# veronicaguerrini/BFQzip

Measured on AMD Instinct MI355X. Metric: Mbases/s end-to-end (eBWT+cluster+LF), reads and results resident in HBM, higher is better.
Workload: dtype u64

## Files before the change

### bfqzip_amd/_lib.py

```python
import ctypes as C
import os
import subprocess

_HERE = os.path.dirname(os.path.abspath(__file__))
LIB_PATH = os.path.join(_HERE, "libbfqhip.so")
_LIB = None

SYMBOLS = [
    "bfq_default_params", "bfq_create", "bfq_create_error", "bfq_destroy", "bfq_set_params",
    "bfq_last_error", "bfq_stream", "bfq_device_count", "bfq_pick_device", "bfq_device_lease", "bfq_device_release",
    "bfq_phase_enable", "bfq_phase", "bfq_phase_report", "bfq_output_prefault", "bfq_fastq_rows_estimate", "bfq_build_ebwt", "bfq_count_reads",
    "bfq_smooth_invert", "bfq_run_reads", "bfq_run_reads_device", "bfq_fetch_ebwt",
    "bfq_fastq_out_bound", "bfq_fastq_build_ebwt", "bfq_fastq_run", "bfq_fastq_run_streams",
    "bfq_smooth_invert_fastq", "bfq_fastq_run_job", "bfq_host_alloc", "bfq_host_free",
    "bfq_text_count_lines", "bfq_text_nth_newline", "bfq_file_put", "bfq_file_map", "bfq_file_unmap", "bfq_fastq_build_ebwt_fd", "bfq_smooth_invert_fastq_fd",
    "bfq_glob_begin", "bfq_glob_local_text", "bfq_glob_pile_counts", "bfq_glob_init_out", "bfq_glob_run_pile", "bfq_glob_finish",
    "bfq_synth_default", "bfq_synth_total", "bfq_synth_host", "bfq_synth_device", "bfq_synth_fastq",
    "bfq_posbin_geometry", "bfq_radix_geometry", "bfq_refine_form", "bfq_prof_enable", "bfq_prof_reset", "bfq_prof_count", "bfq_prof_get", "bfq_prof_trace_select", "bfq_prof_trace",
    "bfq_stream_bound", "bfq_stream_raw_len", "bfq_stream_compress", "bfq_stream_decompress",
    "bfq_stream_reserve", "bfq_stream_compress_device", "bfq_stream_ebwt_decode",
    "bfq_names_compress", "bfq_names_compress_device",
    "bfq_quals_compress", "bfq_quals_compress_device",
    "bfq_fastq_restore_bound", "bfq_fastq_restore", "bfq_fastq_restore_fd",
    "bfq_reorder_key", "bfq_fastq_reorder", "bfq_fastq_reorder_fd",
    "bfq_perm_bound", "bfq_perm_reads", "bfq_perm_encode", "bfq_perm_decode",
    "bfq_fastq_reorder_keep", "bfq_fastq_reorder_keep_fd", "bfq_fastq_unreorder", "bfq_fastq_unreorder_fd",
    "bfq_fastq_restore_ordered", "bfq_fastq_restore_ordered_fd",
    "bfq_fastq_restore_groups", "bfq_stream_members", "bfq_fastq_restore_grouped", "bfq_fastq_restore_grouped_fd",
    "bfq_fastq_compare", "bfq_fastq_compare_fd",
    "bfq_bgzf_probe", "bfq_bgzf_index", "bfq_bgzf_inflate", "bfq_bgzf_inflate_device", "bfq_bgzf_inflate_fd",
    "bfq_bgzf_deflate_bound", "bfq_bgzf_deflate_host", "bfq_bgzf_deflate", "bfq_bgzf_deflate_device", "bfq_bgzf_deflate_fd",
    "bfq_fastq_restore_bgzf_fd",
    "bfq_gzip_probe", "bfq_gzip_measure", "bfq_gzip_inflate", "bfq_gzip_inflate_device", "bfq_gzip_inflate_fd", "bfq_gzip_inflate_host",
    "bfq_gzip_host_error",
    "bfq_bam_default_opts", "bfq_bam_probe", "bfq_bam_measure", "bfq_bam_to_fastq", "bfq_bam_to_fastq_device", "bfq_bam_to_fastq_fd",
    "bfq_bam_to_fastq_host", "bfq_bam_host_error",
    "bfq_bam_patch_host", "bfq_bam_patch_device", "bfq_bam_patch", "bfq_bam_patch_fd",
    "bfq_ubam_default_opts", "bfq_fastq_to_bam_measure", "bfq_fastq_to_bam_host", "bfq_ubam_host_error", "bfq_fastq_to_bam_device", "bfq_fastq_to_bam",
    "bfq_fastq_to_bam_fd", "bfq_fastq_restore_bam_fd",
    "bfq_pairs_default_opts", "bfq_pairs_host_error",
    "bfq_fastq_deinterleave_measure", "bfq_fastq_deinterleave", "bfq_fastq_deinterleave_device", "bfq_fastq_deinterleave_fd", "bfq_fastq_deinterleave_host",
    "bfq_fastq_interleave_measure", "bfq_fastq_interleave", "bfq_fastq_interleave_device", "bfq_fastq_interleave_fd", "bfq_fastq_interleave_host",
    "bfq_repair_default_opts", "bfq_fastq_repair_measure", "bfq_fastq_repair", "bfq_fastq_repair_device", "bfq_fastq_repair_fd", "bfq_fastq_repair_host",
    "bfq_workspace_bytes", "bfq_workspace_read", "bfq_version",
]


class Params(C.Structure):
    _fields_ = [(k, C.c_int32) for k in ("K", "m", "v", "f", "t", "term", "M", "B", "ext", "piles", "ws_cap_mib")] + \
               [("reserved", C.c_int32 * 5)]

# ... 352 lines not shown
        L.bfq_fastq_to_bam_measure.argtypes = [vp, C.POINTER(vp), a3, puo, pu64, a3, pus]
        L.bfq_fastq_to_bam_host.argtypes = [C.POINTER(vp), a3, puo, vp, u64, pu64, pus]
        L.bfq_fastq_to_bam_device.argtypes = [vp, C.POINTER(vp), a3, puo, vp, u64, pu64, pus]
        L.bfq_fastq_to_bam.argtypes = [vp, C.POINTER(vp), a3, puo, vp, u64, pu64, pus]
        L.bfq_fastq_to_bam_fd.argtypes = [vp, i3, puo, C.c_int, pu64, pus]
        L.bfq_fastq_restore_bam_fd.argtypes = [vp, C.c_int, u64, C.c_int, u64, C.c_int, u64, C.c_int, u64, puo, C.c_int, pu64, pus]
        ppo, pps2 = C.POINTER(PairsOpts), C.POINTER(PairsStats)
        L.bfq_pairs_default_opts.restype = None
        L.bfq_pairs_default_opts.argtypes = [ppo]
        L.bfq_pairs_host_error.restype = C.c_char_p
        L.bfq_pairs_host_error.argtypes = []
        L.bfq_fastq_deinterleave_measure.argtypes = [vp, vp, u64, ppo, a3, a3, pps2]
        L.bfq_fastq_deinterleave.argtypes = [vp, vp, u64, ppo, C.POINTER(vp), a3, a3, a3, pps2]
        L.bfq_fastq_deinterleave_device.argtypes = [vp, vp, u64, ppo, C.POINTER(vp), a3, a3, a3, pps2]
        L.bfq_fastq_deinterleave_fd.argtypes = [vp, C.c_int, u64, ppo, i3, a3, a3, pps2]
        L.bfq_fastq_deinterleave_host.argtypes = [vp, u64, ppo, C.POINTER(vp), a3, a3, a3, pps2]
        L.bfq_fastq_interleave_measure.argtypes = [vp, C.POINTER(vp), a3, ppo, pu64, a3, pps2]
        L.bfq_fastq_interleave.argtypes = [vp, C.POINTER(vp), a3, ppo, vp, u64, pu64, pps2]
        L.bfq_fastq_interleave_device.argtypes = [vp, C.POINTER(vp), a3, ppo, vp, u64, pu64, pps2]
        L.bfq_fastq_interleave_fd.argtypes = [vp, i3, ppo, C.c_int, pu64, pps2]
        L.bfq_fastq_interleave_host.argtypes = [C.POINTER(vp), a3, ppo, vp, u64, pu64, pps2]
        pro, prs = C.POINTER(RepairOpts), C.POINTER(RepairStats)
        L.bfq_repair_default_opts.restype = None
        L.bfq_repair_default_opts.argtypes = [pro]
        L.bfq_fastq_repair_measure.argtypes = [vp, C.POINTER(vp), a3, pro, a3, a3, prs]
        L.bfq_fastq_repair.argtypes = [vp, C.POINTER(vp), a3, pro, C.POINTER(vp), a3, a3, a3, prs]
        L.bfq_fastq_repair_device.argtypes = [vp, C.POINTER(vp), a3, pro, C.POINTER(vp), a3, a3, a3, prs]
        L.bfq_fastq_repair_fd.argtypes = [vp, i3, pro, i3, a3, a3, prs]
        L.bfq_fastq_repair_host.argtypes = [C.POINTER(vp), a3, pro, C.POINTER(vp), a3, a3, a3, prs]
        L.bfq_fastq_restore_bgzf_fd.argtypes = [vp, C.c_int, u64, C.c_int, u64, C.c_int, u64, C.c_int, u64, C.c_int, C.c_int, pu64, pu64, pu64]
        L.bfq_posbin_geometry.argtypes = [u64, C.POINTER(u64), C.POINTER(C.c_int)]
        L.bfq_radix_geometry.argtypes = [u64, C.POINTER(u64), C.POINTER(u64)]
        L.bfq_refine_form.argtypes = [vp]
        L.bfq_prof_enable.argtypes = [vp, C.c_int]
        L.bfq_prof_reset.argtypes = [vp]
        L.bfq_prof_count.argtypes = [vp]
        L.bfq_prof_trace_select.argtypes = [vp, C.c_int]
        L.bfq_prof_trace.restype = C.c_int64
        L.bfq_prof_trace.argtypes = [vp, vp, u64]
        L.bfq_prof_get.argtypes = [vp, C.c_int, C.c_char_p, C.c_int, C.POINTER(C.c_double),
                                   C.POINTER(u64), C.POINTER(C.c_double)]
        _LIB = L
    return _LIB
```

### bfqzip_amd/api.py

```python
import ctypes as C
import numpy as np
from . import _lib


class BfqError(RuntimeError):
    def __init__(self, code, msg):
        super().__init__(f"libbfqhip error {code}: {msg}")
        self.code = code


def make_params(k=16, m=2, v=ord(">"), f=40, t=20, s=ord("#"), M=2, B=0, ext=0, piles=0, ws_cap_mib=0):
    p = _lib.Params()
    p.K, p.m, p.v, p.f, p.t, p.term, p.M, p.B, p.ext, p.piles, p.ws_cap_mib = k, m, v, f, t, s, M, B, ext, piles, ws_cap_mib
    return p


def _ptr(a):
    return C.c_void_p(a.ctypes.data) if a is not None else None


def _u8(text):
    if isinstance(text, np.ndarray):
        return text if (text.dtype == np.uint8 and text.flags.c_contiguous) else np.ascontiguousarray(text, np.uint8)
    return np.frombuffer(text, np.uint8)
# ... 1270 lines not shown

    @staticmethod
    def perm_encode(perm, mode=0, k=0, seed=0):
        return perm_encode(perm, mode=mode, k=k, seed=seed)

    @staticmethod
    def perm_decode(permz):
        return perm_decode(permz)

    def stream_compress_device(self, d_in, n, d_out, cap):
        ol = C.c_uint64(0)
        self._ck(self.L.bfq_stream_compress_device(self.h, d_in, n, d_out, cap, C.byref(ol)))
        return int(ol.value)

    def names_compress_device(self, d_in, n, d_out, cap, always=False):
        ol = C.c_uint64(0)
        self._ck(self.L.bfq_names_compress_device(self.h, d_in, n, 1 if always else 0, d_out, cap, C.byref(ol)))
        return int(ol.value)

    def quals_compress_device(self, d_in, n, d_out, cap, always=False, rung=None):
        ol = C.c_uint64(0)
        self._ck(self.L.bfq_quals_compress_device(self.h, d_in, n, self._quals_flags(always, rung), d_out, cap, C.byref(ol)))
        return int(ol.value)

    def stream_reserve(self, n):
        self._ck(self.L.bfq_stream_reserve(self.h, n))

    def stream_bound(self, n):
        return int(self.L.bfq_stream_bound(n))

    def refine_form(self):
        return int(self.L.bfq_refine_form(self.h))

    def prof_reset(self):
        self.L.bfq_prof_reset(self.h)

    def prof(self):
        out = {}
        name = C.create_string_buffer(64)
        for i in range(self.L.bfq_prof_count(self.h)):
            ms = C.c_double(); ln = C.c_uint64(); by = C.c_double()
            self.L.bfq_prof_get(self.h, i, name, 64, C.byref(ms), C.byref(ln), C.byref(by))
            if ln.value:
                out[name.value.decode()] = {"ms": ms.value, "launches": ln.value, "alg_bytes": by.value}
        return out

    def prof_trace_select(self, kernel):
        name = C.create_string_buffer(64)
        idx = -1
        for i in range(self.L.bfq_prof_count(self.h)):
            self.L.bfq_prof_get(self.h, i, name, 64, None, None, None)
            if kernel is not None and name.value.decode() == kernel:
                idx = i
        if kernel is not None and idx < 0:
            raise KeyError(kernel)
        self._ck(self.L.bfq_prof_trace_select(self.h, idx))

    def prof_trace(self):
        k = int(self.L.bfq_prof_trace(self.h, None, 0))
        out = np.empty(max(k, 0), np.float32)
        if k > 0:
            self.L.bfq_prof_trace(self.h, _ptr(out), k)
        return out

    def workspace_bytes(self):
        return int(self.L.bfq_workspace_bytes(self.h))
# ... 74 lines not shown
```

### bfqzip_amd/csrc/bfq_api.hip

```cpp
#include <math.h>
#include <time.h>
#include <stdlib.h>
#include <stdio.h>
#include <string.h>
#include <unistd.h>
#include <errno.h>
#include <algorithm>
#include <new>
#include "bfq_internal.h"
#include "bfq_synth.h"
#include "bfq_device.h"
#include "bfq_rank.h"
#include "bfq_posbin.h"

const char *const BFQ_KERNEL_NAMES[K_NUM] = {
    "k_text_from_reads", "k_pack3", "k_build_keys", "k_radix_hist", "k_scan", "k_radix_scatter", "k_huge_round",
    "k_cluster_big", "k_refine_chunk", "k_refine_big", "k_emit_bwt", "k_lf_count", "k_lf_build", "k_lcp_flags",
    "k_cluster", "k_invert_count", "k_invert", "k_synth", "k_fastq", "k_bfs", "k_codec", "misc",
    "k_restore_index", "k_fq_format_lines", "k_reorder_keys", "k_reorder_gather",
    "k_fq_format_ordered", "k_perm_pack", "k_perm_invert", "k_posbin_l1", "k_posbin_l2", "k_posbin_apply", "k_posbin_check",
    "k_cmp_check", "k_cmp_compare", "k_cmp_emit", "k_bgzf_inflate", "k_bgzf_deflate", "k_ubam_size", "k_ubam_write", "k_pairs_cmp", "k_pairs_move"};

static thread_local std::string g_createErr;

// ... 240 lines not shown
    if (!c) return;
    memset(c->profMs, 0, sizeof c->profMs); memset(c->profLaunches, 0, sizeof c->profLaunches);
    memset(c->profBytes, 0, sizeof c->profBytes);
    c->profTrace.clear();
}
extern "C" int bfq_prof_trace_select(bfq_ctx *c, int idx)
{
    if (!c || idx < -1 || idx >= K_NUM) return BFQ_E_ARG;
    c->profTraceId = idx; c->profTrace.clear();
    return BFQ_OK;
}
extern "C" int64_t bfq_prof_trace(bfq_ctx *c, float *ms, uint64_t cap)
{
    if (!c) return BFQ_E_ARG;
    const size_t k = std::min<size_t>(cap, c->profTrace.size());
    if (ms && k) memcpy(ms, c->profTrace.data(), k * sizeof(float));
    return (int64_t)c->profTrace.size();
}
extern "C" int bfq_prof_count(bfq_ctx *c) { (void)c; return K_NUM; }
extern "C" int bfq_posbin_geometry(uint64_t n_rows, uint64_t *window, int *bin_shift)
{
    const int s = bfq_posbin_shift(n_rows);
    if (window) *window = BFQ_PB_W;
    if (bin_shift) *bin_shift = s;
    return s >= 0 ? BFQ_OK : BFQ_E_ARG;
}
extern "C" int bfq_radix_geometry(uint64_t n_rows, uint64_t *tile_rows, uint64_t *block_rows)
{
    if (tile_rows) *tile_rows = BFQ_RS_TILE;
    if (block_rows) *block_rows = bfq_radix_block_elems(n_rows);
    return BFQ_OK;
}
extern "C" int bfq_refine_form(bfq_ctx *c) { return c ? (c->env.refinePipe ? 1 : 0) : BFQ_E_ARG; }
extern "C" int bfq_prof_get(bfq_ctx *c, int idx, char *name, int cap, double *ms, uint64_t *launches, double *bytes)
{
    if (!c || idx < 0 || idx >= K_NUM) return BFQ_E_ARG;
    if (name && cap > 0) { strncpy(name, BFQ_KERNEL_NAMES[idx], cap - 1); name[cap - 1] = 0; }
    if (ms) *ms = c->profMs[idx];
    if (launches) *launches = c->profLaunches[idx];
    if (bytes) *bytes = c->profBytes[idx];
    return BFQ_OK;
}

static void check_counters(bfq_ctx *c)
{
    const DevCounters &h = c->h_cnt;
    if (h.errSymbol) throw BfqError{BFQ_E_SYMBOL, "symbol outside {A,C,G,T,N,terminator}"};
    if (h.errTooLong) throw BfqError{BFQ_E_TOO_LONG, "read longer than BFQ_MAX_READ_LEN"};
    if (h.errInvert) throw BfqError{BFQ_E_NOT_EBWT, "LF walk did not close: not an eBWT of a read collection"};
    if (h.mismatch) throw BfqError{BFQ_E_NOT_EBWT, "eBWT is not in #_i<#_j<A<C<G<N<T suffix order"};
    if (h.errFreq3) throw BfqError{BFQ_E_FREQ3, "three frequent symbols in a cluster (bfq_int.cpp:505 assert); raise -f"};
}
static void finish_call(bfq_ctx *c, bfq_stats *st = nullptr)
{
    c->fetchCounters();
    c->profCollect();
    check_counters(c);
    if (!st) return;
    const u64 *s = c->h_cnt.stats;
    st->num_clust = s[0]; st->num_clust_discarded = s[1]; st->num_clust_amb_discarded = s[2];
    st->num_clust_mod = s[3]; st->num_clust_alleq = s[4]; st->bases_inside = s[5];
    st->qs_smoothed = s[6]; st->modified = s[7];
    st->n_rows = c->n; st->n_reads = c->N;
    st->n_segments = c->h_cnt.nSegs; st->n_big_segments = c->h_cnt.bigTotal + c->h_cnt.bigCount;
}

// ... 1258 lines not shown
```

### bfqzip_amd/csrc/bfq_host.cpp

```cpp
#include <errno.h>
#include <fcntl.h>
#include <stdio.h>
#include <stdlib.h>
#include <string.h>
#include <sched.h>
#include <sys/file.h>
#include <sys/mman.h>
#include <sys/stat.h>
#include <time.h>
#include <unistd.h>
#include <algorithm>
#include <atomic>
#include <condition_variable>
#include <mutex>
#include <string>
#include <thread>
#include <vector>
#include "bfq_internal_host.h"
#include "bfq_reorder.h"
#include "bfq_perm.h"
#include "bfq_bgzf.h"

static double now_s()
{
    struct timespec ts;
    clock_gettime(CLOCK_MONOTONIC, &ts);
    return ts.tv_sec + 1e-9 * ts.tv_nsec;
}

BfqEnv bfq_env_read()
{
    {
        BfqEnv e;
        auto geti = [](const char *k, int dflt) { const char *v = getenv(k); return (v && *v) ? atoi(v) : dflt; };
        auto getu = [](const char *k, unsigned long long dflt) {
            const char *v = getenv(k);
            if (!v || !*v) return dflt;
            char *end = nullptr;
            double x = strtod(v, &end);
            if (end && (*end == 'G' || *end == 'g')) x *= 1073741824.0;
            else if (end && (*end == 'M' || *end == 'm')) x *= 1048576.0;
            else if (end && (*end == 'K' || *end == 'k')) x *= 1024.0;
            return (unsigned long long)x;
        };
        e.trace = getenv("BFQ_TRACE") != nullptr;
        e.piles = getenv("BFQ_PILES") ? (atoi(getenv("BFQ_PILES")) == 2 ? 2 : atoi(getenv("BFQ_PILES")) ? 1 : -1) : 0;
        e.pilesSplit = getenv("BFQ_PILES_SPLIT") != nullptr;
        e.noOverlap = getenv("BFQ_NO_OVERLAP") != nullptr;
        e.noLengthGuess = getenv("BFQ_NO_LENGTH_GUESS") != nullptr;
        e.posMode = geti("BFQ_POSMODE", 0) != 0;
        e.posBins = geti("BFQ_POSBINS", 1) != 0;
        e.posBinWc = geti("BFQ_POSBIN_WC", 1) != 0;
        e.fuseKeys = geti("BFQ_FUSEKEYS", 1) != 0;
        e.refinePipe = geti("BFQ_REFINE_PIPE", 1) != 0;
        e.ioThreads = geti("BFQ_IO_THREADS", 0);
        e.prefaultThreads = geti("BFQ_PREFAULT_THREADS", -1);
        e.hugeCap = getu("BFQ_HUGE_CAP", 0);
        e.wsCap = getu("BFQ_WS_CAP", 0);
        e.device = getenv("BFQ_DEVICE") ? atoi(getenv("BFQ_DEVICE")) : -1;
        e.fakeDevices = geti("BFQ_FAKE_DEVICES", 0);
        e.lease = geti("BFQ_LEASE", 1) != 0;
        if (const char *d = getenv("BFQ_LEASE_DIR")) e.leaseDir = d;
        e.noOutmap = getenv("BFQ_NO_OUTMAP") != nullptr;
        e.compact = geti("BFQ_COMPACT", 0) != 0;
        if (const char *v = getenv("BFQ_POISON")) {
            char *end = nullptr;
            const long b = strtol(v, &end, 0);
            if (*v && end && !*end && b >= 0 && b <= 255) e.poison = (int)b;
        }
        e.prefaultPause = geti("BFQ_PREFAULT_PAUSE", 0) != 0;
        e.compactWin = getu("BFQ_COMPACT_WIN", 0);
        e.compactRing = getu("BFQ_COMPACT_RING", 0);
        e.bgzfBatch = getu("BFQ_BGZF_BATCH", 0);
        e.dnaStatic = geti("BFQ_DNA_STATIC", 0);
        e.dnacK = geti("BFQ_DNAC_K", 0); e.dnacH = geti("BFQ_DNAC_H", 0); e.dnacW = geti("BFQ_DNAC_W", 0); e.dnacSkip = geti("BFQ_DNAC_TSKIP", -1);
        return e;
    }
}
const BfqEnv &bfq_env()
{
    static const BfqEnv E = bfq_env_read();
    return E;
}

int bfq_cpu_budget()
{
    static const int budget = [] {
// ... 523 lines not shown
```

### bfqzip_amd/csrc/bfq_internal_host.h

```cpp
#pragma once
#include <stdint.h>
#include <sys/mman.h>
#include <atomic>
#include <new>
#include <string>
#include "../../include/bfqzip_hip.h"
#include "bfq_common.h"

struct BfqError {
    int code;
    std::string msg;
};

template <class F> static int host_guarded(std::string &err, F body)
{
    err.clear();
    try {
        body();
        return BFQ_OK;
    } catch (const BfqError &e) {
        err = e.msg;
        return e.code;
    } catch (const std::bad_alloc &) {
        err = "host out of memory";
        return BFQ_E_NOMEM;
    }
}
static inline void zero3(uint64_t *a) { if (a) a[0] = a[1] = a[2] = 0; }

struct MappedInput {
    void *p = MAP_FAILED; size_t n = 0;
    MappedInput() = default;
    MappedInput(const MappedInput &) = delete; MappedInput &operator=(const MappedInput &) = delete;
    bool open(int fd, size_t len) { n = len; p = len ? mmap(nullptr, len, PROT_READ, MAP_PRIVATE, fd, 0) : MAP_FAILED; return !len || p != MAP_FAILED; }
    const uint8_t *data() const { return p != MAP_FAILED ? (const uint8_t *)p : nullptr; }
    ~MappedInput() { if (p != MAP_FAILED) munmap(p, n); }
};

struct BfqEnv {
    bool trace = false;
    int piles = 0;
    bool pilesSplit = false;
    bool noOverlap = false;
    bool noLengthGuess = false;
    bool posMode = false;
    bool posBins = true;
    bool posBinWc = true;
    bool fuseKeys = true;
    bool refinePipe = true;
    int ioThreads = 0;
    int prefaultThreads = -1;
    unsigned long long hugeCap = 0;
    unsigned long long wsCap = 0;
    int device = -1;
    int fakeDevices = 0;
    bool lease = true;
    std::string leaseDir;
    bool compact = false;
    int dnaStatic = 0;
    int dnacK = 0, dnacH = 0, dnacW = 0, dnacSkip = -1;
    unsigned long long compactRing = 0;
    unsigned long long compactWin = 0;
    bool prefaultPause = false;
    unsigned long long bgzfBatch = 0;
    int poison = -1;
    bool noOutmap = false;
};
BfqEnv bfq_env_read();
const BfqEnv &bfq_env();
int bfq_cpu_budget();
extern std::atomic<bool> g_bfqHipStarted;
extern std::atomic<int> g_bfqUploadsRunning;

struct bfq_outmap;
bfq_outmap *bfq_outmap_open(int fd, uint64_t map_len, uint64_t prefault_len);
bfq_outmap *bfq_outmap_take(int fd, uint64_t min_len);
char *bfq_outmap_ptr(bfq_outmap *m);
uint64_t bfq_outmap_len(bfq_outmap *m);
void bfq_outmap_extend(bfq_outmap *m, uint64_t prefault_len);
bool bfq_outmap_close(bfq_outmap *m, uint64_t final_len);
bool bfq_outmap_ensure(bfq_outmap *m, uint64_t off, uint64_t len);
int bfq_outmap_fd(bfq_outmap *m);
// ... 9 lines not shown
```

### bfqzip_amd/csrc/k_cluster.hip

```cpp
#include <stdlib.h>
#include "bfq_internal.h"
#include "bfq_device.h"
#include "bfq_rank.h"
#include "bfq_rankblk.h"

__global__ __launch_bounds__(256) void k_lcp_flags(const u16 *__restrict__ lcp, u64 n, int K, u8 *__restrict__ in)
{
    const u64 ngroups = (n + 7) / 8;
    for (u64 g = (u64)blockIdx.x * blockDim.x + threadIdx.x; g < ngroups; g += (u64)gridDim.x * blockDim.x) {
        u64 r0 = g * 8;
        int l[10];
        if (r0 >= 1 && r0 + 9 <= n) {
            u64 a = *(const u64 *)(lcp + r0 - 1), b = *(const u64 *)(lcp + r0 + 3);
            u32 c = *(const u32 *)(lcp + r0 + 7);
#pragma unroll
            for (int k = 0; k < 4; k++) { l[k] = (int)((a >> (16 * k)) & 0xFFFF); l[4 + k] = (int)((b >> (16 * k)) & 0xFFFF); }
            l[8] = (int)(c & 0xFFFF); l[9] = (int)(c >> 16);
        } else {
#pragma unroll
            for (int k = 0; k < 10; k++) { u64 r = r0 + k; l[k] = (r >= 1 && r - 1 < n) ? (int)lcp[r - 1] : 0; }
        }
        u64 out = 0;
#pragma unroll
        for (int k = 0; k < 8; k++) {
            u64 r = r0 + k;
            bool thr = (r >= 1) && (l[k + 1] >= K);
            bool mn = (r >= 1 && r + 2 <= n) && (l[k] > l[k + 1]) && (l[k + 2] >= l[k + 1]);
            out |= (u64)((thr && !mn) ? 1 : 0) << (8 * k);
        }
        if (r0 + 8 <= n) *(u64 *)(in + r0) = out;
        else for (u64 r = r0; r < n; r++) in[r] = (u8)(out >> (8 * (r - r0)));
    }
}

struct ClStat { u32 clust, disc, amb, mod, alleq, bases, qs, modb; };

struct BigState;
struct ClusterArgs {
    RankIndex R;
    const u8 *bwt; const u8 *qual; const u8 *in; u64 n;
    int m, v, f, t, term, M, ext;
    const double *powtab;
    const double *qthr;
    int qthrLo, qthrN;
    DevCounters *cnt;
    const u64 *w12;
    const u64 *text3;
    u8 *outSym, *outQual;
    int B;
    const u64 *rankBlk;
    u64 F[6];
    u8 *editQual, *repl;
    u64 *bigStart;
    struct BigState *big;
    u16 *firstOut;
};

__device__ __forceinline__ int ord5(u8 c)
{
    return c == 'A' ? 0 : c == 'C' ? 1 : c == 'G' ? 2 : c == 'T' ? 3 : 4;
}
__device__ __forceinline__ u8 dna5(int i) { return (u8)((0x4E54474341ull >> (8 * i)) & 0xFF); }

__device__ __forceinline__ u64 row_pos(const ClusterArgs &a, u64 j)
{
    const u64 x = a.w12[j];
    return bfq_val_pos(bfq_rec_pay((u32)x, (u32)(x >> 32)));
}
__device__ __forceinline__ void set_qual(const ClusterArgs &a, u64 j, int newqs)
{
    if (a.w12 && a.outQual) { const u32 q = (u32)newqs & 0xFFu; a.outQual[row_pos(a, j) - 1] = (u8)(a.B ? bfq_bin8(q) : q); }
    else if (a.w12 || a.rankBlk) a.editQual[j] = (u8)newqs;
    else lfq_set_qual(a.R.lfq, j, (u32)newqs & 0xFFu);
}
__device__ __forceinline__ void set_mod(const ClusterArgs &a, u64 j, u8 sym)
{
    if (a.w12 && a.outSym) a.outSym[row_pos(a, j) - 1] = sym;
    else if (a.w12 || a.rankBlk) a.repl[j] = sym;
    else lfq_set_repl(a.R.lfq, j, bfq_base_code(a.bwt[j]), bfq_base_code(sym));
}
__device__ __forceinline__ u8 prec_sym(const ClusterArgs &a, u64 j)
{
    if (a.rankBlk) {
        const RankBlk b = load_blk(a.rankBlk, j >> 6);
        const u32 code = blk_code(b, j);
        if (!code) return (u8)a.term;
        return a.bwt[a.F[code] + blk_occ_of(b, j, code)];
    }
    if (!a.w12) return a.bwt[lfq_next(a.R.lfq[j])];
    const u64 p = row_pos(a, j);
    if (p < 2) return (u8)a.term;
    const u64 t = p - 2, w = t / BFQ_SYMS_PER_WORD;
    const u32 code = (u32)(a.text3[bfq_t3_at(w)] >> (3u * (20u - (u32)(t - w * BFQ_SYMS_PER_WORD)))) & 7u;
    return code ? bfq_code_sym(code) : (u8)a.term;
}

__device__ __forceinline__ void mod_smooth(const ClusterArgs &a, u64 start, u64 end, u8 newSymb, int newqs, u32 lowQS, ClStat &st)
{
    const u8 TERM = (u8)a.term;
    for (u64 j0 = start; j0 <= end; j0 += 8) {
        u64 xb = *(const u64 *)(a.bwt + j0), xq = *(const u64 *)(a.qual + j0);
        u32 cnt = (end - j0 + 1 < 8) ? (u32)(end - j0 + 1) : 8u;
        for (u32 k = 0; k < cnt; k++) {
            u64 j = j0 + k;
            u8 b = (u8)(xb >> (8 * k));
            if (b == TERM) continue;
            if (b != newSymb && !((lowQS >> ord5(b)) & 1u)) { set_mod(a, j, newSymb); st.modb++; }
            else if (b == newSymb) { set_qual(a, j, newqs); st.qs++; }
            else if (newqs < (int)(signed char)(u8)(xq >> (8 * k))) { set_qual(a, j, newqs); st.qs++; }
        }
    }
}

#define CL_BIG 2048
__device__ __forceinline__ bool process_cluster_body(const ClusterArgs &a, u64 start, ClStat &st)
{
    const u8 TERM = (u8)a.term;
    u32 freqs[5] = {0, 0, 0, 0, 0};
    u32 lowQS = 0;
    u64 base_num = 0;
    int sum = 0, mx = 0;
    double sum_err = 0;
// ... 65 lines not shown
    if (Freq[0] == 'N') { mod_smooth(a, start, end, Freq[1], newqs, lowQS, st); st.mod++; return false; }
    if (Freq[1] == 'N') { mod_smooth(a, start, end, Freq[0], newqs, lowQS, st); st.mod++; return false; }

    u8 symbPrec[2] = {0, 0};
    u32 fr[2] = {0, 0};
    for (u64 j = start; j <= end; j++) {
        u8 b = a.bwt[j];
        int w = (b == Freq[0]) ? 0 : ((b == Freq[1]) ? 1 : -1);
        if (w < 0) continue;
        u8 ch = prec_sym(a, j);
        if (ch != TERM && ch != 'N') { fr[w] |= 1u << ord5(ch); symbPrec[w] = ch; }
    }
    if (__popc(fr[0] & 15u) == 1 && __popc(fr[1] & 15u) == 1 && symbPrec[0] != symbPrec[1]) {
        st.mod++;
        for (u64 j = start; j <= end; j++) {
            u8 b = a.bwt[j];
            if (b == TERM) continue;
            if (b != Freq[0] && b != Freq[1] && !((lowQS >> ord5(b)) & 1u)) {
                u8 ch = prec_sym(a, j);
                if (ch == symbPrec[0]) { set_mod(a, j, Freq[0]); st.modb++; }
                else if (ch == symbPrec[1]) { set_mod(a, j, Freq[1]); st.modb++; }
            } else if (b == Freq[0] || b == Freq[1]) {
                set_qual(a, j, newqs); st.qs++;
            } else if (newqs < (int)(signed char)a.qual[j]) {
                set_qual(a, j, newqs); st.qs++;
            }
        }
    } else {
        st.amb++;
    }
    return false;
}

#define CL_CHUNK 4096
#define CL_WROWS (CL_CHUNK / 4)
__global__ __launch_bounds__(256) void k_cluster(ClusterArgs a, u64 nchunks)
{
    __shared__ u32 shst[8];
    __shared__ u16 starts[4][CL_WROWS];
    __shared__ u32 wn[4];
    const u32 lane = bfq_lane(), w = threadIdx.x >> 6;
    if (threadIdx.x < 8) shst[threadIdx.x] = 0;
    ClStat st = {0, 0, 0, 0, 0, 0, 0, 0};
    for (u64 ch = blockIdx.x; ch < nchunks; ch += gridDim.x) {
        const u64 r0 = ch * CL_CHUNK + (u64)w * CL_WROWS + (u64)lane * (CL_WROWS / 64);
        u32 bits = 0;
        if (r0 < a.n) {
            uint4 x = *(const uint4 *)(a.in + r0);
            u32 wds[4] = {x.x, x.y, x.z, x.w};
#pragma unroll
            for (int q = 0; q < 4; q++)
#pragma unroll
                for (int b = 0; b < 4; b++) bits |= ((wds[q] >> (8 * b)) & 1u) << (4 * q + b);
            if (r0 + 16 > a.n) bits &= (1u << (u32)(a.n - r0)) - 1u;
        }
        {
            const u32 zb = ~bits & 0xFFFFu;
            const u64 any = __ballot(zb != 0);
            const int fl = any ? __builtin_ctzll(any) : -1;
            const u32 fz = (u32)__builtin_amdgcn_readlane((int)zb, fl < 0 ? 0 : fl);
            if (lane == 0) a.firstOut[ch * 4 + w] = (u16)(fl < 0 ? CL_WROWS : fl * (CL_WROWS / 64) + __builtin_ctz(fz));
        }
        u32 prev = (r0 >= 1 && r0 < a.n) ? (u32)a.in[r0 - 1] & 1u : 0u;
        u32 sb = bits & ~((bits << 1) | prev) & 0xFFFFu;
        u32 ns = (u32)__popc(sb);
        u32 incl = bfq_wave_incscan32(ns);
        u32 o = incl - ns;
        while (sb) { u32 k = (u32)__builtin_ctz(sb); starts[w][o++] = (u16)(w * CL_WROWS + lane * (CL_WROWS / 64) + k); sb &= sb - 1; }
        u32 cntw = (u32)__builtin_amdgcn_readlane((int)incl, 63);
        if (lane == 0) wn[w] = cntw;
        __syncthreads();
        u32 n0 = wn[0], n1 = wn[1], n2 = wn[2], n3 = wn[3];
        u32 total = n0 + n1 + n2 + n3;
        for (u32 t = threadIdx.x; t < total; t += 256) {
            u32 ww = t < n0 ? 0u : (t < n0 + n1 ? 1u : (t < n0 + n1 + n2 ? 2u : 3u));
            u32 idx = t - (ww == 0 ? 0u : (ww == 1 ? n0 : (ww == 2 ? n0 + n1 : n0 + n1 + n2)));
            u64 r = ch * CL_CHUNK + starts[ww][idx];
            if (process_cluster_body(a, r - 1, st)) a.bigStart[atomicAdd(&a.cnt->bigClusters, 1ull)] = r;
        }
        __syncthreads();
    }
    if (st.clust) atomicAdd(&shst[0], st.clust);
    if (st.disc) atomicAdd(&shst[1], st.disc);
    if (st.amb) atomicAdd(&shst[2], st.amb);
    if (st.mod) atomicAdd(&shst[3], st.mod);
    if (st.alleq) atomicAdd(&shst[4], st.alleq);
    if (st.bases) atomicAdd(&shst[5], st.bases);
    if (st.qs) atomicAdd(&shst[6], st.qs);
    if (st.modb) atomicAdd(&shst[7], st.modb);
    __syncthreads();
    if (threadIdx.x < 8 && shst[threadIdx.x]) atomicAdd(&a.cnt->stats[threadIdx.x], (u64)shst[threadIdx.x]);
}

struct BigState {
    u64 start, end;
    u64 freq[5];
    u32 low, sum, mx, fr0, fr1;
    int mode, newqs;
    u32 sym0, sym1;
};
#define CB_TILE 65536
#define CB_GRID 2048

#define CB_FOR_ROWS(...)                                                                               \
    for (u64 g0 = (ts & ~15ull) + (u64)threadIdx.x * 16; g0 <= te; g0 += 256 * 16) {                  \
        const uint4 xb4 = *(const uint4 *)(a.bwt + g0), xq4 = *(const uint4 *)(a.qual + g0);          \
        const u32 xbw[4] = {xb4.x, xb4.y, xb4.z, xb4.w}, xqw[4] = {xq4.x, xq4.y, xq4.z, xq4.w};        \
        _Pragma("unroll") for (int k = 0; k < 16; k++) {                                              \
            const u64 j = g0 + k;                                                                      \
            if (j < ts || j > te) continue;                                                            \
            const u8 b = (u8)(xbw[k >> 2] >> (8 * (k & 3)));                                           \
// ... 186 lines not shown
                        else if (newqs < (int)(signed char)qb) { set_qual(a, j, newqs); qs++; }
                    })
            }
        })
    if (qs) atomicAdd(&a.cnt->stats[6], (u64)qs);
    if (modb) atomicAdd(&a.cnt->stats[7], (u64)modb);
}

void bfq_lcp_flags(bfq_ctx *c, const u16 *lcp, u64 n, int K, u8 *in)
{
    if (!n) return;
    KLAUNCH(c, K_LCP_FLAGS, 3.0 * (double)n, k_lcp_flags, bfq_grid((n + 7) / 8, 256), 256, lcp, n, K, in);
}

void bfq_clusters(bfq_ctx *c, const RankIndex &R, const u8 *bwt, const u8 *qual, const u8 *in, u64 n, const ClusterPos *pm,
                  const ClusterRank *rm)
{
    if (!n) return;
    ClusterArgs a;
    a.R = R; a.bwt = bwt; a.qual = qual; a.in = in; a.n = n;
    a.rankBlk = rm ? rm->rankBlk : nullptr; a.editQual = rm ? rm->qual : pm ? pm->editQual : nullptr; a.repl = rm ? rm->repl : pm ? pm->repl : nullptr;
    for (int s = 0; s < 6; s++) a.F[s] = rm ? rm->F[s] : 0;
    a.w12 = pm ? pm->w12 : nullptr; a.text3 = pm ? pm->text3 : nullptr;
    a.outSym = pm ? pm->outSym : nullptr; a.outQual = pm ? pm->outQual : nullptr; a.B = pm ? pm->B : 0;
    a.m = c->P.m; a.v = c->P.v; a.f = c->P.f; a.t = c->P.t; a.term = c->P.term & 0xFF; a.M = c->P.M; a.ext = c->P.ext;
    a.powtab = c->d_powtab; a.qthr = c->d_qthr; a.qthrLo = c->qthrLo; a.qthrN = c->qthrN;
    a.cnt = c->d_cnt;
    size_t mk = c->mark();
    HIP_CHECK(hipMemsetAsync(&c->d_cnt->bigClusters, 0, sizeof(u64), c->stream));
    a.bigStart = c->alloc<u64>(n / CL_BIG + 2);
    a.big = c->alloc<BigState>(n / CL_BIG + 2);
    a.firstOut = c->alloc<u16>(n / CL_WROWS + 8);
    u64 nchunks = ceil_div(n, CL_CHUNK);
    KLAUNCH(c, K_CLUSTER, 4.125 * (double)n, k_cluster, bfq_grid(nchunks, 1), 256, a, nchunks);
    KLAUNCH(c, K_CLUSTER_BIG, 0.0, k_big_extent, 1024, 256, a);
    KLAUNCH(c, K_CLUSTER_BIG, 0.0, k_big_count, CB_GRID, 256, a);
    KLAUNCH(c, K_CLUSTER_BIG, 0.0, k_big_decide, 64, 256, a);
    KLAUNCH(c, K_CLUSTER_BIG, 0.0, k_big_prec, CB_GRID, 256, a);
    KLAUNCH(c, K_CLUSTER_BIG, 0.0, k_big_apply, CB_GRID, 256, a);
    c->release(mk);
}
```

### include/bfqzip_hip.h

```cpp
#ifndef BFQZIP_HIP_H
#define BFQZIP_HIP_H
#include <stdint.h>
#ifdef __cplusplus
extern "C" {
#endif

#define BFQ_OK              0
#define BFQ_E_ARG          -1
#define BFQ_E_HIP          -2
#define BFQ_E_SYMBOL       -3
#define BFQ_E_NOT_EBWT     -4
#define BFQ_E_TOO_LONG     -5
#define BFQ_E_FREQ3        -6
#define BFQ_E_NOMEM        -7
#define BFQ_E_IO           -8

#define BFQ_MAX_READ_LEN 65000

typedef struct bfq_params {
    int32_t K;
    int32_t m;
    int32_t v;
    int32_t f;
    int32_t t;
// ... 310 lines not shown
int bfq_fastq_interleave_host(const uint8_t *const text[3], const uint64_t text_len[3], const bfq_pairs_opts *opts, uint8_t *out, uint64_t cap,
                              uint64_t *out_len, bfq_pairs_stats *stats);
const char *bfq_pairs_host_error(void);
typedef struct bfq_repair_opts  { uint32_t mate_suffix, hash_bits; uint64_t seed; uint32_t reserved[2]; } bfq_repair_opts;
typedef struct bfq_repair_stats { uint64_t records, pairs, singles, out_len[3], n_in[3], dup_groups, mixed_runs, max_run; } bfq_repair_stats;
void bfq_repair_default_opts(bfq_repair_opts *o);
int bfq_fastq_repair_measure(bfq_ctx *c, const uint8_t *const h_text[3], const uint64_t text_len[3], const bfq_repair_opts *opts, uint64_t out_len[3],
                             uint64_t n_reads[3], bfq_repair_stats *stats);
int bfq_fastq_repair(bfq_ctx *c, const uint8_t *const h_text[3], const uint64_t text_len[3], const bfq_repair_opts *opts, uint8_t *const h_out[3],
                     const uint64_t cap[3], uint64_t out_len[3], uint64_t n_reads[3], bfq_repair_stats *stats);
int bfq_fastq_repair_device(bfq_ctx *c, const uint8_t *const d_text[3], const uint64_t text_len[3], const bfq_repair_opts *opts, uint8_t *const d_out[3],
                            const uint64_t cap[3], uint64_t out_len[3], uint64_t n_reads[3], bfq_repair_stats *stats);
int bfq_fastq_repair_fd(bfq_ctx *c, const int text_fd[3], const bfq_repair_opts *opts, const int out_fd[3], uint64_t out_len[3], uint64_t n_reads[3],
                        bfq_repair_stats *stats);
int bfq_fastq_repair_host(const uint8_t *const text[3], const uint64_t text_len[3], const bfq_repair_opts *opts, uint8_t *const h_out[3],
                          const uint64_t cap[3], uint64_t out_len[3], uint64_t n_reads[3], bfq_repair_stats *stats);
uint64_t bfq_bgzf_deflate_bound(uint64_t len);
int bfq_bgzf_deflate_host(const uint8_t *h_in, uint64_t len, int level, uint8_t *h_out, uint64_t cap, uint64_t *out_len);
int bfq_bgzf_deflate(bfq_ctx *c, const uint8_t *h_in, uint64_t len, int level, uint8_t *h_out, uint64_t cap, uint64_t *out_len);
int bfq_bgzf_deflate_device(bfq_ctx *c, const uint8_t *d_in, uint64_t len, int level, uint8_t *h_out, uint64_t cap, uint64_t *out_len);
int bfq_bgzf_deflate_fd(bfq_ctx *c, int in_fd, uint64_t len, int level, int out_fd, uint64_t *out_len);
int bfq_fastq_restore_bgzf_fd(bfq_ctx *c, int dna_fd, uint64_t dna_len, int qs_fd, uint64_t qs_len, int hdr_fd, uint64_t hdr_len,
                              int perm_fd, uint64_t permz_len, int level, int out_fd, uint64_t *out_len, uint64_t *raw_len,
                              uint64_t *n_reads);
int bfq_stream_reserve(bfq_ctx *c, uint64_t len);
int bfq_stream_compress_device(bfq_ctx *c, const uint8_t *d_in, uint64_t len, uint8_t *d_out, uint64_t cap, uint64_t *out_len);

int  bfq_prof_enable(bfq_ctx *c, int on);
void bfq_prof_reset(bfq_ctx *c);
int  bfq_prof_count(bfq_ctx *c);
int  bfq_posbin_geometry(uint64_t n_rows, uint64_t *window, int *bin_shift);
int  bfq_radix_geometry(uint64_t n_rows, uint64_t *tile_rows, uint64_t *block_rows);
int  bfq_refine_form(bfq_ctx *c);
int  bfq_prof_get(bfq_ctx *c, int idx, char *name, int name_cap, double *total_ms,
                  uint64_t *launches, double *alg_bytes_total);
int     bfq_prof_trace_select(bfq_ctx *c, int idx);
int64_t bfq_prof_trace(bfq_ctx *c, float *ms, uint64_t cap);

uint64_t bfq_workspace_bytes(bfq_ctx *c);
uint64_t bfq_workspace_read(bfq_ctx *c, uint64_t off, void *dst, uint64_t len);
const char *bfq_version(void);

#ifdef __cplusplus
}
#endif
#endif
```

Baseline: 11710.

## Process cluster rows eight at a time with SWAR byte masks and mode-specialized kernels

Adds a SWAR path for the cluster kernel. It loads 8 BWT, quality and LCP-flag bytes as one u64 and computes base counts, quality sums, max, threshold tests and edit masks with bitwise tricks instead of a per-row loop. The kernel is templated on output mode and quality method, so the per-row pointer-null branches in set_qual, set_mod and prec_sym fold away at compile time. In local mode, edits are written as blended 8-byte stores. This adds unaligned 64-bit loads that can read past the cluster end, a float-reciprocal division with a correction step, and eight kernel instantiations; it can be turned off with BFQ_CLUSTER8.

```diff
diff --git a/bfqzip_amd/_lib.py b/bfqzip_amd/_lib.py
--- a/bfqzip_amd/_lib.py
+++ b/bfqzip_amd/_lib.py
@@ -16,7 +16,7 @@
     "bfq_text_count_lines", "bfq_text_nth_newline", "bfq_file_put", "bfq_file_map", "bfq_file_unmap", "bfq_fastq_build_ebwt_fd", "bfq_smooth_invert_fastq_fd",
     "bfq_glob_begin", "bfq_glob_local_text", "bfq_glob_pile_counts", "bfq_glob_init_out", "bfq_glob_run_pile", "bfq_glob_finish",
     "bfq_synth_default", "bfq_synth_total", "bfq_synth_host", "bfq_synth_device", "bfq_synth_fastq",
-    "bfq_posbin_geometry", "bfq_radix_geometry", "bfq_refine_form", "bfq_prof_enable", "bfq_prof_reset", "bfq_prof_count", "bfq_prof_get", "bfq_prof_trace_select", "bfq_prof_trace",
+    "bfq_posbin_geometry", "bfq_radix_geometry", "bfq_refine_form", "bfq_cluster_form", "bfq_prof_enable", "bfq_prof_reset", "bfq_prof_count", "bfq_prof_get", "bfq_prof_trace_select", "bfq_prof_trace",
     "bfq_stream_bound", "bfq_stream_raw_len", "bfq_stream_compress", "bfq_stream_decompress",
     "bfq_stream_reserve", "bfq_stream_compress_device", "bfq_stream_ebwt_decode",
     "bfq_names_compress", "bfq_names_compress_device",
@@ -435,6 +435,7 @@
         L.bfq_posbin_geometry.argtypes = [u64, C.POINTER(u64), C.POINTER(C.c_int)]
         L.bfq_radix_geometry.argtypes = [u64, C.POINTER(u64), C.POINTER(u64)]
         L.bfq_refine_form.argtypes = [vp]
+        L.bfq_cluster_form.argtypes = [vp]
         L.bfq_prof_enable.argtypes = [vp, C.c_int]
         L.bfq_prof_reset.argtypes = [vp]
         L.bfq_prof_count.argtypes = [vp]
diff --git a/bfqzip_amd/api.py b/bfqzip_amd/api.py
--- a/bfqzip_amd/api.py
+++ b/bfqzip_amd/api.py
@@ -1326,6 +1326,9 @@
     def refine_form(self):
         return int(self.L.bfq_refine_form(self.h))
 
+    def cluster_form(self):
+        return int(self.L.bfq_cluster_form(self.h))
+
     def prof_reset(self):
         self.L.bfq_prof_reset(self.h)
 
diff --git a/bfqzip_amd/csrc/bfq_api.hip b/bfqzip_amd/csrc/bfq_api.hip
--- a/bfqzip_amd/csrc/bfq_api.hip
+++ b/bfqzip_amd/csrc/bfq_api.hip
@@ -296,6 +296,7 @@
     return BFQ_OK;
 }
 extern "C" int bfq_refine_form(bfq_ctx *c) { return c ? (c->env.refinePipe ? 1 : 0) : BFQ_E_ARG; }
+extern "C" int bfq_cluster_form(bfq_ctx *c) { return c ? (c->env.cluster8 ? 1 : 0) : BFQ_E_ARG; }
 extern "C" int bfq_prof_get(bfq_ctx *c, int idx, char *name, int cap, double *ms, uint64_t *launches, double *bytes)
 {
     if (!c || idx < 0 || idx >= K_NUM) return BFQ_E_ARG;
diff --git a/bfqzip_amd/csrc/bfq_cluster8.h b/bfqzip_amd/csrc/bfq_cluster8.h
--- /dev/null
+++ b/bfqzip_amd/csrc/bfq_cluster8.h
@@ -0,0 +1,97 @@
+#pragma once
+#include "bfq_common.h"
+
+#define BFQ_CL8_H 0x8080808080808080ull
+#define BFQ_CL8_7 0x7F7F7F7F7F7F7F7Full
+
+struct BfqCl8Acc { u32 fA, fC, fG, fT, fN, bases, lowQS; int sum, mx; };
+
+BFQ_HD u64 bfq_cl8_rep(u32 c)
+{
+    const u32 r = (c & 0xFFu) * 0x01010101u;
+    return ((u64)r << 32) | r;
+}
+BFQ_HD u64 bfq_cl8_zero(u64 y)
+{
+    return ~(((y & BFQ_CL8_7) + BFQ_CL8_7) | y) & BFQ_CL8_H;
+}
+BFQ_HD u64 bfq_cl8_eq(u64 x, u32 c) { return bfq_cl8_zero(x ^ bfq_cl8_rep(c)); }
+BFQ_HD u64 bfq_cl8_rows(u32 cnt)
+{
+    return cnt >= 8u ? BFQ_CL8_H : (BFQ_CL8_H & ((1ull << (8u * cnt)) - 1ull));
+}
+BFQ_HD u64 bfq_cl8_bytes(u64 f) { return f | (f - (f >> 7)); }
+BFQ_HD u64 bfq_cl8_blend(u64 f, u32 c, u64 x)
+{
+    const u64 m = bfq_cl8_bytes(f);
+    return (bfq_cl8_rep(c) & m) | (x & ~m);
+}
+
+BFQ_HD u64 bfq_cl8_ge(u64 xq, int thr)
+{
+    if (thr <= -128) return BFQ_CL8_H;
+    if (thr > 127) return 0;
+    const u64 x = xq ^ BFQ_CL8_H;
+    const u64 y = bfq_cl8_rep((u32)(thr + 128));
+    const u64 d = (x | BFQ_CL8_H) - (y & BFQ_CL8_7);
+    return ((x & ~y) | (~(x ^ y) & d)) & BFQ_CL8_H;
+}
+
+BFQ_HD u32 bfq_cl8_div(u32 num, u32 den, float rden)
+{
+    u32 q = (u32)((float)num * rden);
+    const u32 r = num - q * den;
+    if ((int)r < 0) q--;
+    else if (r >= den) q++;
+    return q;
+}
+
+struct BfqCl8Sym { u64 base, nA, nC, nG, nT, nN; };
+BFQ_HD BfqCl8Sym bfq_cl8_symbols(u64 xb, u32 cnt, u32 term)
+{
+    BfqCl8Sym s;
+    s.base = bfq_cl8_rows(cnt) & ~bfq_cl8_eq(xb, term);
+    s.nA = bfq_cl8_eq(xb, 'A') & s.base; s.nC = bfq_cl8_eq(xb, 'C') & s.base;
+    s.nG = bfq_cl8_eq(xb, 'G') & s.base; s.nT = bfq_cl8_eq(xb, 'T') & s.base;
+    s.nN = s.base & ~(s.nA | s.nC | s.nG | s.nT);
+    return s;
+}
+
+BFQ_HD void bfq_cl8_count(u64 xb, u64 xq, u32 cnt, u32 term, int thr, BfqCl8Acc *acc)
+{
+    const BfqCl8Sym s = bfq_cl8_symbols(xb, cnt, term);
+    const u32 nb = (u32)bfq_popc64(s.base);
+    acc->fA += (u32)bfq_popc64(s.nA); acc->fC += (u32)bfq_popc64(s.nC); acc->fG += (u32)bfq_popc64(s.nG);
+    acc->fT += (u32)bfq_popc64(s.nT); acc->fN += (u32)bfq_popc64(s.nN);
+    acc->bases += nb;
+    const u64 pass = bfq_cl8_ge(xq, thr);
+    acc->lowQS |= ((pass & s.nA) ? 1u : 0u) | ((pass & s.nC) ? 2u : 0u) | ((pass & s.nG) ? 4u : 0u) | ((pass & s.nT) ? 8u : 0u) |
+                  ((pass & s.nN) ? 16u : 0u);
+    const u64 bm = bfq_cl8_bytes(s.base);
+    const u64 u = (xq ^ BFQ_CL8_H) & bm;
+    const u64 s4 = (u & 0x00FF00FF00FF00FFull) + ((u >> 8) & 0x00FF00FF00FF00FFull);
+    const u32 s2 = (u32)s4 + (u32)(s4 >> 32);
+    acc->sum = (int)((u32)acc->sum + (s2 & 0xFFFFu) + (s2 >> 16) - 128u * nb);
+    u64 p = xq & bm;
+    p &= ~bfq_cl8_bytes(p & BFQ_CL8_H);
+    const u32 lo = (u32)p, hi = (u32)(p >> 32);
+    u32 m = (u32)acc->mx;
+    for (int k = 0; k < 4; k++) {
+        const u32 a = (lo >> (8 * k)) & 0xFFu, b = (hi >> (8 * k)) & 0xFFu;
+        m = a > m ? a : m;
+        m = b > m ? b : m;
+    }
+    acc->mx = (int)m;
+}
+
+BFQ_HD void bfq_cl8_edit(u64 xb, u64 xq, u32 cnt, u32 term, u32 newSymb, u32 lowQS, int newqs, u64 *modMask, u64 *qualMask)
+{
+    const BfqCl8Sym s = bfq_cl8_symbols(xb, cnt, term);
+    const u64 trusted = ((lowQS & 1u) ? s.nA : 0ull) | ((lowQS & 2u) ? s.nC : 0ull) | ((lowQS & 4u) ? s.nG : 0ull) |
+                        ((lowQS & 8u) ? s.nT : 0ull) | ((lowQS & 16u) ? s.nN : 0ull);
+    const u64 same = bfq_cl8_eq(xb, newSymb) & s.base;
+    const u64 other = s.base & ~same;
+    const u64 above = newqs >= 127 ? 0ull : bfq_cl8_ge(xq, newqs + 1);
+    *modMask = other & ~trusted;
+    *qualMask = same | (other & trusted & above);
+}
diff --git a/bfqzip_amd/csrc/bfq_host.cpp b/bfqzip_amd/csrc/bfq_host.cpp
--- a/bfqzip_amd/csrc/bfq_host.cpp
+++ b/bfqzip_amd/csrc/bfq_host.cpp
@@ -53,6 +53,7 @@
         e.posBinWc = geti("BFQ_POSBIN_WC", 1) != 0;
         e.fuseKeys = geti("BFQ_FUSEKEYS", 1) != 0;
         e.refinePipe = geti("BFQ_REFINE_PIPE", 1) != 0;
+        e.cluster8 = geti("BFQ_CLUSTER8", 1) != 0;
         e.ioThreads = geti("BFQ_IO_THREADS", 0);
         e.prefaultThreads = geti("BFQ_PREFAULT_THREADS", -1);
         e.hugeCap = getu("BFQ_HUGE_CAP", 0);
diff --git a/bfqzip_amd/csrc/bfq_internal_host.h b/bfqzip_amd/csrc/bfq_internal_host.h
--- a/bfqzip_amd/csrc/bfq_internal_host.h
+++ b/bfqzip_amd/csrc/bfq_internal_host.h
@@ -48,6 +48,7 @@
     bool posBinWc = true;
     bool fuseKeys = true;
     bool refinePipe = true;
+    bool cluster8 = true;
     int ioThreads = 0;
     int prefaultThreads = -1;
     unsigned long long hugeCap = 0;
diff --git a/bfqzip_amd/csrc/k_cluster.hip b/bfqzip_amd/csrc/k_cluster.hip
--- a/bfqzip_amd/csrc/k_cluster.hip
+++ b/bfqzip_amd/csrc/k_cluster.hip
@@ -3,6 +3,7 @@
 #include "bfq_device.h"
 #include "bfq_rank.h"
 #include "bfq_rankblk.h"
+#include "bfq_cluster8.h"
 
 __global__ __launch_bounds__(256) void k_lcp_flags(const u16 *__restrict__ lcp, u64 n, int K, u8 *__restrict__ in)
 {
@@ -67,27 +68,36 @@
     const u64 x = a.w12[j];
     return bfq_val_pos(bfq_rec_pay((u32)x, (u32)(x >> 32)));
 }
-__device__ __forceinline__ void set_qual(const ClusterArgs &a, u64 j, int newqs)
-{
-    if (a.w12 && a.outQual) { const u32 q = (u32)newqs & 0xFFu; a.outQual[row_pos(a, j) - 1] = (u8)(a.B ? bfq_bin8(q) : q); }
-    else if (a.w12 || a.rankBlk) a.editQual[j] = (u8)newqs;
+enum { CLM_ROWS = -1, CLM_LF = 0, CLM_POS = 1, CLM_LOCAL = 2, CLM_RANK = 3 };
+__host__ __device__ __forceinline__ int cluster_mode(const ClusterArgs &a)
+{
+    return a.rankBlk ? CLM_RANK : !a.w12 ? CLM_LF : (a.outSym || a.outQual) ? CLM_POS : CLM_LOCAL;
+}
+template <int MODE = CLM_ROWS> __device__ __forceinline__ void set_qual(const ClusterArgs &a, u64 j, int newqs)
+{
+    const bool pos = MODE == CLM_ROWS ? (a.w12 && a.outQual) : (MODE == CLM_POS && a.outQual);
+    const bool loc = MODE == CLM_ROWS ? (a.w12 || a.rankBlk) : MODE != CLM_LF;
+    if (pos) { const u32 q = (u32)newqs & 0xFFu; a.outQual[row_pos(a, j) - 1] = (u8)(a.B ? bfq_bin8(q) : q); }
+    else if (loc) a.editQual[j] = (u8)newqs;
     else lfq_set_qual(a.R.lfq, j, (u32)newqs & 0xFFu);
 }
-__device__ __forceinline__ void set_mod(const ClusterArgs &a, u64 j, u8 sym)
-{
-    if (a.w12 && a.outSym) a.outSym[row_pos(a, j) - 1] = sym;
-    else if (a.w12 || a.rankBlk) a.repl[j] = sym;
+template <int MODE = CLM_ROWS> __device__ __forceinline__ void set_mod(const ClusterArgs &a, u64 j, u8 sym)
+{
+    const bool pos = MODE == CLM_ROWS ? (a.w12 && a.outSym) : (MODE == CLM_POS && a.outSym);
+    const bool loc = MODE == CLM_ROWS ? (a.w12 || a.rankBlk) : MODE != CLM_LF;
+    if (pos) a.outSym[row_pos(a, j) - 1] = sym;
+    else if (loc) a.repl[j] = sym;
     else lfq_set_repl(a.R.lfq, j, bfq_base_code(a.bwt[j]), bfq_base_code(sym));
 }
-__device__ __forceinline__ u8 prec_sym(const ClusterArgs &a, u64 j)
-{
-    if (a.rankBlk) {
+template <int MODE = CLM_ROWS> __device__ __forceinline__ u8 prec_sym(const ClusterArgs &a, u64 j)
+{
+    if (MODE == CLM_ROWS ? a.rankBlk != nullptr : MODE == CLM_RANK) {
         const RankBlk b = load_blk(a.rankBlk, j >> 6);
         const u32 code = blk_code(b, j);
         if (!code) return (u8)a.term;
         return a.bwt[a.F[code] + blk_occ_of(b, j, code)];
     }
-    if (!a.w12) return a.bwt[lfq_next(a.R.lfq[j])];
+    if (MODE == CLM_ROWS ? !a.w12 : MODE == CLM_LF) return a.bwt[lfq_next(a.R.lfq[j])];
     const u64 p = row_pos(a, j);
     if (p < 2) return (u8)a.term;
     const u64 t = p - 2, w = t / BFQ_SYMS_PER_WORD;
@@ -219,9 +229,140 @@
     return false;
 }
 
+template <int MODE>
+__device__ __forceinline__ void mod_smooth8(const ClusterArgs &a, u64 start, u64 end, u8 newSymb, int newqs, u32 lowQS, ClStat &st)
+{
+    for (u64 j0 = start; j0 <= end; j0 += 8) {
+        const u64 xb = *(const u64 *)(a.bwt + j0), xq = *(const u64 *)(a.qual + j0);
+        const u32 cnt = (end - j0 + 1 < 8) ? (u32)(end - j0 + 1) : 8u;
+        u64 mm, qm;
+        bfq_cl8_edit(xb, xq, cnt, (u32)a.term, newSymb, lowQS, newqs, &mm, &qm);
+        st.modb += (u32)__popcll(mm); st.qs += (u32)__popcll(qm);
+        if (MODE == CLM_LOCAL || MODE == CLM_RANK) {
+            if (cnt == 8u) {
+                if (qm) *(u64 *)(a.editQual + j0) = bfq_cl8_blend(qm, (u32)newqs, xq);
+                if (mm) *(u64 *)(a.repl + j0) = bfq_cl8_blend(mm, newSymb, 0);
+            } else {
+                for (u64 f = qm; f; f &= f - 1) a.editQual[j0 + ((u32)__builtin_ctzll(f) >> 3)] = (u8)newqs;
+                for (u64 f = mm; f; f &= f - 1) a.repl[j0 + ((u32)__builtin_ctzll(f) >> 3)] = newSymb;
+            }
+        } else {
+            for (u64 f = mm; f; f &= f - 1) set_mod<MODE>(a, j0 + ((u32)__builtin_ctzll(f) >> 3), newSymb);
+            for (u64 f = qm; f; f &= f - 1) set_qual<MODE>(a, j0 + ((u32)__builtin_ctzll(f) >> 3), newqs);
+        }
+    }
+}
+
+template <int MODE, int MSEL>
+__device__ __forceinline__ bool process_cluster8(const ClusterArgs &a, u64 start, ClStat &st)
+{
+    const int M = MSEL < 0 ? a.M : MSEL;
+    const u8 TERM = (u8)a.term;
+    BfqCl8Acc acc = {0, 0, 0, 0, 0, 0, 0, 0, 0};
+    const int thr = a.t + 33;
+    double sum_err = 0;
+    u64 end;
+    for (u64 j0 = start;; j0 += 8) {
+        const u64 xin = *(const u64 *)(a.in + j0 + 1);
+        const u64 z = (xin - 0x0101010101010101ull) & ~xin & 0x8080808080808080ull;
+        u32 run = z ? (u32)(__builtin_ctzll(z) >> 3) : 8u;
+        if (j0 + run >= a.n) run = (u32)(a.n - 1 - j0);
+        const u32 cnt = run < 8 ? run + 1 : 8u;
+        const u64 xb = *(const u64 *)(a.bwt + j0), xq = *(const u64 *)(a.qual + j0);
+        bfq_cl8_count(xb, xq, cnt, (u32)TERM, thr, &acc);
+        if (M == 1)
+            for (u32 k = 0; k < cnt; k++)
+                if ((u8)(xb >> (8 * k)) != TERM) sum_err = sum_err + a.powtab[(u8)(xq >> (8 * k))];
+        if (run < 8) { end = j0 + run; break; }
+        if (j0 + 8 - start >= CL_BIG) return true;
+    }
+    const u32 size = (u32)(end - start) + 1u;
+    const u32 base_num = acc.bases;
+    const bool counted = (u64)size >= (u64)(long long)a.m;
+    st.clust += counted ? 1u : 0u;
+    if (!counted || base_num == 0) return false;
+    st.bases += base_num;
+    const float rbase = 1.0f / (float)base_num;
+
+    int newqs;
+    if (M == 1) {
+        double avg_err = sum_err / (double)base_num;
+        int lo = 0, hi = a.qthrN - 1;
+        while (lo < hi) { int mid = (lo + hi) >> 1; if (a.qthr[mid] <= avg_err) hi = mid; else lo = mid + 1; }
+        int q = a.qthrLo + lo;
+        newqs = a.ext ? (int)(signed char)(u8)((u8)q + 33) : (int)(signed char)(q + 33);
+    } else if (M == 2) {
+        newqs = (int)(signed char)a.v;
+    } else if (M == 3) {
+        const int sum = acc.sum;
+        if (sum == 0) newqs = 0;
+        else if (a.ext) newqs = (int)(signed char)(u8)roundf((float)sum / (float)base_num);
+        else if (sum > 0) newqs = (int)(signed char)(int)bfq_cl8_div((u32)sum, base_num, rbase);
+        else newqs = (int)(signed char)(int)((u64)(long long)sum / (u64)base_num);
+    } else {
+        newqs = acc.mx;
+    }
+
+    u32 F0 = 0, F1 = 0;
+    u32 nf = 0, nnn = 0;
+#define CL8_FREQ(fr, sym)                                                                  \
+    {                                                                                      \
+        const u32 perc = bfq_cl8_div(100u * (fr), base_num, rbase) & 0xFFu;                \
+        const bool hit = (fr) > 0 && (float)perc >= (float)a.f;                            \
+        nnn += (fr) > 0 ? 1u : 0u;                                                         \
+        F1 = (hit && nf == 1) ? (u32)(sym) : F1;                                           \
+        F0 = (hit && nf == 0) ? (u32)(sym) : F0;                                           \
+        nf += hit ? 1u : 0u;                                                               \
+    }
+    CL8_FREQ(acc.fA, 'A') CL8_FREQ(acc.fC, 'C') CL8_FREQ(acc.fG, 'G') CL8_FREQ(acc.fT, 'T') CL8_FREQ(acc.fN, 'N')
+#undef CL8_FREQ
+    const u32 lowQS = acc.lowQS;
+    st.alleq += nnn == 1 ? 1u : 0u;
+    if (nf >= 3) { atomicAdd(&a.cnt->errFreq3, 1ull); return false; }
+    const bool few = (u64)base_num < (u64)(long long)a.m;
+    const bool pair = nf == 2 && !few;
+    const bool two = pair && F0 != 'N' && F1 != 'N';
+    st.disc += (nf == 0 || (nf == 1 && F0 == 'N') || (nf == 2 && few)) ? 1u : 0u;
+    st.mod += (pair && !two) ? 1u : 0u;
+    const u32 target = nf == 1 ? (F0 == 'N' ? 0u : F0) : (pair && !two) ? (F0 == 'N' ? F1 : F0) : 0u;
+    if (target) { mod_smooth8<MODE>(a, start, end, (u8)target, newqs, lowQS, st); return false; }
+    if (!two) return false;
+
+    u8 prec0 = 0, prec1 = 0;
+    u32 fr0 = 0, fr1 = 0;
+    for (u64 j = start; j <= end; j++) {
+        const u8 b = a.bwt[j];
+        if (b != (u8)F0 && b != (u8)F1) continue;
+        const u8 ch = prec_sym<MODE>(a, j);
+        if (ch != TERM && ch != 'N') {
+            if (b == (u8)F0) { fr0 |= 1u << ord5(ch); prec0 = ch; }
+            else { fr1 |= 1u << ord5(ch); prec1 = ch; }
+        }
+    }
+    if (__popc(fr0 & 15u) == 1 && __popc(fr1 & 15u) == 1 && prec0 != prec1) {
+        st.mod++;
+        for (u64 j = start; j <= end; j++) {
+            const u8 b = a.bwt[j];
+            if (b == TERM) continue;
+            if (b != (u8)F0 && b != (u8)F1 && !((lowQS >> ord5(b)) & 1u)) {
+                const u8 ch = prec_sym<MODE>(a, j);
+                if (ch == prec0) { set_mod<MODE>(a, j, (u8)F0); st.modb++; }
+                else if (ch == prec1) { set_mod<MODE>(a, j, (u8)F1); st.modb++; }
+            } else if (b == (u8)F0 || b == (u8)F1) {
+                set_qual<MODE>(a, j, newqs); st.qs++;
+            } else if (newqs < (int)(signed char)a.qual[j]) {
+                set_qual<MODE>(a, j, newqs); st.qs++;
+            }
+        }
+    } else {
+        st.amb++;
+    }
+    return false;
+}
+
 #define CL_CHUNK 4096
 #define CL_WROWS (CL_CHUNK / 4)
-__global__ __launch_bounds__(256) void k_cluster(ClusterArgs a, u64 nchunks)
+template <int MODE, int MSEL> __global__ __launch_bounds__(256) void k_cluster(ClusterArgs a, u64 nchunks)
 {
     __shared__ u32 shst[8];
     __shared__ u16 starts[4][CL_WROWS];
@@ -263,7 +404,9 @@
             u32 ww = t < n0 ? 0u : (t < n0 + n1 ? 1u : (t < n0 + n1 + n2 ? 2u : 3u));
             u32 idx = t - (ww == 0 ? 0u : (ww == 1 ? n0 : (ww == 2 ? n0 + n1 : n0 + n1 + n2)));
             u64 r = ch * CL_CHUNK + starts[ww][idx];
-            if (process_cluster_body(a, r - 1, st)) a.bigStart[atomicAdd(&a.cnt->bigClusters, 1ull)] = r;
+            bool big;
+            if constexpr (MODE == CLM_ROWS) big = process_cluster_body(a, r - 1, st); else big = process_cluster8<MODE, MSEL>(a, r - 1, st);
+            if (big) a.bigStart[atomicAdd(&a.cnt->bigClusters, 1ull)] = r;
         }
         __syncthreads();
     }
@@ -516,7 +659,14 @@
     a.big = c->alloc<BigState>(n / CL_BIG + 2);
     a.firstOut = c->alloc<u16>(n / CL_WROWS + 8);
     u64 nchunks = ceil_div(n, CL_CHUNK);
-    KLAUNCH(c, K_CLUSTER, 4.125 * (double)n, k_cluster, bfq_grid(nchunks, 1), 256, a, nchunks);
+    int mode = c->env.cluster8 ? cluster_mode(a) : CLM_ROWS;
+    if (mode == CLM_LOCAL) mode = 4 + ((a.M >= 1 && a.M <= 3) ? a.M : 0);
+    switch (mode) {
+#define CL_LAUNCH(ID, MODE, MSEL) case ID: KLAUNCH(c, K_CLUSTER, 4.125 * (double)n, (k_cluster<MODE, MSEL>), bfq_grid(nchunks, 1), 256, a, nchunks); break;
+    CL_LAUNCH(CLM_ROWS, CLM_ROWS, -1) CL_LAUNCH(CLM_LF, CLM_LF, -1) CL_LAUNCH(CLM_POS, CLM_POS, -1) CL_LAUNCH(CLM_RANK, CLM_RANK, -1)
+    CL_LAUNCH(4, CLM_LOCAL, 0) CL_LAUNCH(5, CLM_LOCAL, 1) CL_LAUNCH(6, CLM_LOCAL, 2) CL_LAUNCH(7, CLM_LOCAL, 3)
+#undef CL_LAUNCH
+    }
     KLAUNCH(c, K_CLUSTER_BIG, 0.0, k_big_extent, 1024, 256, a);
     KLAUNCH(c, K_CLUSTER_BIG, 0.0, k_big_count, CB_GRID, 256, a);
     KLAUNCH(c, K_CLUSTER_BIG, 0.0, k_big_decide, 64, 256, a);
diff --git a/include/bfqzip_hip.h b/include/bfqzip_hip.h
--- a/include/bfqzip_hip.h
+++ b/include/bfqzip_hip.h
@@ -366,6 +366,7 @@
 int  bfq_posbin_geometry(uint64_t n_rows, uint64_t *window, int *bin_shift);
 int  bfq_radix_geometry(uint64_t n_rows, uint64_t *tile_rows, uint64_t *block_rows);
 int  bfq_refine_form(bfq_ctx *c);
+int  bfq_cluster_form(bfq_ctx *c);
 int  bfq_prof_get(bfq_ctx *c, int idx, char *name, int name_cap, double *total_ms,
                   uint64_t *launches, double *alg_bytes_total);
 int     bfq_prof_trace_select(bfq_ctx *c, int idx);
```

Result: slower. 11440 (-2.3%).
